# xytpai/kfunca

Measured on AMD Instinct MI355X. Metric: bf16 GEMM TFLOP/s + causal-attn fwd+bwd tokens/s, higher is better.
Workload: dtype bf16

## Files before the change

kfunca_amd/csrc/device/attention.hip:

```cpp
#include <math.h>
#include <stdlib.h>

#include <algorithm>
#include <type_traits>

#include "common.h"

namespace kf {

typedef __attribute__((ext_vector_type(8))) __bf16 bf16x8;
typedef __attribute__((ext_vector_type(8))) _Float16 f16x8;
typedef __attribute__((ext_vector_type(4))) short s16x4;
typedef __attribute__((ext_vector_type(8))) short s16x8;
typedef __attribute__((ext_vector_type(16))) float f32x16;
typedef __attribute__((ext_vector_type(4))) float f32x4;

struct AttnArgs {
    const char *q, *k, *v, *o, *d_o;
    char *out, *dq, *dk, *dv;
    float *lse;
    const float *lse_r;
    float *delta;
    float *nlse, *ndelta;
    int64_t B, H, Sq, Skv, D;
// ... 397 lines not shown
    const unsigned long long tl_loop0 = tl_t;
#endif
    for (int t = 0; t < nt; ++t) {
        const int64_t kv0 = (int64_t)t * ABK;
        TL_STAMP(6)
        asm volatile("s_waitcnt vmcnt(4)" ::: "memory");
        TL_STAMP(0)
        __builtin_amdgcn_s_barrier();
        asm volatile("" ::: "memory");
        TL_STAMP(1)
        stage(t + 2, smem + ((t + 2) % SRING) * FBUF);
        TL_STAMP(2)
        const char *cur = smem + (t % SRING) * FBUF;
        const bool skip = !active || kv0 > qw + 31 || KF_MUT(1, t == 1 && qblk == nxb - 1);
        const bool diag = kv0 + ABK - 1 > qw;
        if (late && pending) s_pv<BF, DB>(smem + ((t + SRING - 1) % SRING) * FBUF + FTILE, vo, pf, o);
        pending = false;
        TL_STAMP(5)
        if (!skip) {
            if (diag) s_qk_sm<BF, true, D>(cur, qf, ko, o, pf, m_i, l_i, c, kv0, m, hl, a.defer TL_ARGS);
            else s_qk_sm<BF, false, D>(cur, qf, ko, o, pf, m_i, l_i, c, kv0, m, hl, a.defer TL_ARGS);
            TL_STAMP(4)
            if (late) pending = true;
            else s_pv<BF, DB>(cur + FTILE, vo, pf, o);
            TL_STAMP(5)
        }
    }
#if defined(KF_ATTN_TIMELINE) && KF_ATTN_TIMELINE != 2
    if (lane == 0 && g_attn_tl) {
        unsigned long long *dst = g_attn_tl + ((size_t)blockIdx.x * 2 + (pass & 1)) * 64 + wid * 8;
        for (int i = 0; i < 7; ++i) dst[i] = tl_acc[i];
        dst[7] = (unsigned long long)nt;
    }
#endif
#ifdef KF_ATTN_TIMELINE
    const unsigned long long tl_loop1 = __builtin_amdgcn_s_memtime();
#endif
    if (late && pending) s_pv<BF, DB>(smem + ((nt + SRING - 1) % SRING) * FBUF + FTILE, vo, pf, o);
    asm volatile("s_waitcnt vmcnt(0)" ::: "memory");
    __syncthreads();
    if (active) {
        a_store_rows<BF, DB>(smem + wid * 32 * OPAD, a.out + a_head(a.lo, bh, a.H) + qw * a.lo.sr, o, 1.f / l_i, a.lo.sr);
        if (a.lse && hl == 0) a.lse[bh * a.Sq + m] = (m_i * c + __builtin_amdgcn_logf(l_i)) * kLn2;
    }
    if (a.persist) __syncthreads();
#if defined(KF_ATTN_TIMELINE) && KF_ATTN_TIMELINE == 2
    if (lane == 0 && g_attn_tl) {
        unsigned long long *dst = g_attn_tl + ((size_t)blockIdx.x * 2 + (pass & 1)) * 64 + wid * 8;
        const unsigned long long tl_end = __builtin_amdgcn_s_memtime();
        dst[0] = tl_loop0 - tl_pass0, dst[1] = tl_loop1 - tl_loop0, dst[2] = tl_end - tl_loop1;
        dst[3] = dst[4] = dst[5] = dst[6] = 0;
        dst[7] = (unsigned long long)nt;
    }
#endif
  }
}

#ifndef KF_FWD_W4_INC
#define KF_FWD_W4_INC "attn_fwd_w4.inc"
#endif
#include KF_FWD_W4_INC
template <bool BF, bool SQ, bool D64 = false>
__global__ __launch_bounds__(256) void attn_fwd_w4_kernel(const AttnArgs a) {
    static_assert(!(SQ && D64), "the scaled-query form exists for head size 128 only");
    extern __shared__ __attribute__((aligned(16))) char smem[];
    const int nxb = (int)((a.Sq + FQ - 1) / FQ);
    const int nwx = a.persist ? nxb / 2 : nxb;
    const unsigned lds = (unsigned)(uintptr_t)(const __attribute__((address_space(3))) char *)smem;
    const int wid = __builtin_amdgcn_readfirstlane(threadIdx.x >> 6);
    const int dbytes = D64 ? 128 : 256;
    const unsigned kvn = (unsigned)((a.Skv - 1) * a.lk.sr + dbytes);
    const float c = a.scale_log2e, defer = a.defer;
    const int qsr = (int)a.lq.sr, kvsr = (int)a.lk.sr, osr = (int)a.lo.sr;
#pragma nounroll
    for (unsigned vwg = blockIdx.x; vwg < a.nvwg; vwg += gridDim.x) {
    int xb0;
    int64_t bh;
    a_block_map(nwx, a.nbh, a.xcd_map, xb0, bh, vwg);
    const char *kp = a.k + a_head_kv(a.lk, bh, a.H, a.G), *vp = a.v + a_head_kv(a.lv, bh, a.H, a.G);
    const char *qh = a.q + a_head(a.lq, bh, a.H);
    char *oh = a.out + a_head(a.lo, bh, a.H);
#pragma nounroll
    for (int pass = 0; pass < (a.persist ? 2 : 1); ++pass) {
        const int xb = ((pass & 1) != (a.persist_rev != 0)) ? nxb - 1 - xb0 : xb0;
        const int qblk = nxb - 1 - xb;
        const int64_t q0 = (int64_t)qblk * FQ;
        const char *qp = qh + q0 * a.lq.sr;
        char *op = oh + q0 * a.lo.sr;
        float *lsep = a.lse ? a.lse + bh * a.Sq + q0 : nullptr;
        const int T = (int)((q0 + FQ) / ABK);
        const int64_t qrows = a.Sq - q0 < FQ ? a.Sq - q0 : FQ;
        const unsigned qn = (unsigned)((qrows - 1) * a.lq.sr + dbytes), on = (unsigned)((qrows - 1) * a.lo.sr + dbytes), lsen = (unsigned)(qrows * 4);
        int mut = -1;
#ifdef KF_MUTANT
        if (a.mutant == 1 && qblk == nxb - 1) mut = 1;
#endif
#ifdef KF_FWD_W4_STAMPS
        unsigned long long *dbg = a.dbg;
        const unsigned dbgoff = (vwg * 2 + pass) * 4 * 32;
#define KF_W4_EXTRA , [dbg] "s"(dbg), [dbgoff] "s"(dbgoff)
#else
#define KF_W4_EXTRA
#endif
#define KF_W4_OPERANDS                                                                                                              \
    [qp] "s"(qp), [kp] "s"(kp), [vp] "s"(vp), [op] "s"(op), [lsep] "s"(lsep), [qsr] "s"(qsr), [kvsr] "s"(kvsr), [osr] "s"(osr), [T] "s"(T), \
        [wid] "s"(wid), [c] "s"(c), [defer] "s"(defer), [lds] "s"(lds), [mut] "s"(mut), [kvn] "s"(kvn), [qn] "s"(qn), [on] "s"(on), [lsen] "s"(lsen) KF_W4_EXTRA
        if constexpr (D64 && BF) asm volatile(KF_FWD_W4_D64_ASM_BF16 : : KF_W4_OPERANDS : KF_FWD_W4_CLOBBERS);
        else if constexpr (D64) asm volatile(KF_FWD_W4_D64_ASM_F16 : : KF_W4_OPERANDS : KF_FWD_W4_CLOBBERS);
        else if constexpr (BF && SQ) asm volatile(KF_FWD_W4_ASM_BF16_SQ : : KF_W4_OPERANDS : KF_FWD_W4_CLOBBERS);
        else if constexpr (BF) asm volatile(KF_FWD_W4_ASM_BF16 : : KF_W4_OPERANDS : KF_FWD_W4_CLOBBERS);
        else if constexpr (SQ) asm volatile(KF_FWD_W4_ASM_F16_SQ : : KF_W4_OPERANDS : KF_FWD_W4_CLOBBERS);
        else asm volatile(KF_FWD_W4_ASM_F16 : : KF_W4_OPERANDS : KF_FWD_W4_CLOBBERS);
#undef KF_W4_OPERANDS
#undef KF_W4_EXTRA
    }
    }
}

template <bool BF, int R>
__global__ __launch_bounds__(256) void attn_delta_kernel(const char *o, const char *d_o, float *delta, int64_t nrows, const float *lse, float *nlse,
                                                         float *ndelta, float rscale, AttnArgs::Lay lo, AttnArgs::Lay ldo, int64_t S, int64_t H, int nparts, int64_t Sc) {
    const int64_t row0 = (int64_t)blockIdx.x * (16 * R) + (threadIdx.x >> 4);
    const int part = threadIdx.x & 15;
    uint4 a[R], b[R];
#pragma unroll
    for (int i = 0; i < R; ++i) {
        a[i] = b[i] = uint4{0, 0, 0, 0};
        const int64_t row = row0 + 16 * i;
        const int64_t bh = row / Sc, sq = row - bh * Sc;
        if (row < nrows && sq < S && part < nparts) {
            a[i] = *(const uint4 *)(o + a_head(lo, bh, H) + sq * lo.sr + part * 16);
            b[i] = *(const uint4 *)(d_o + a_head(ldo, bh, H) + sq * ldo.sr + part * 16);
        }
    }
#pragma unroll
    for (int i = 0; i < R; ++i) {
        const int64_t row = row0 + 16 * i;
        float acc = 0.f;
        const uint32_t aw[4] = {a[i].x, a[i].y, a[i].z, a[i].w}, bw[4] = {b[i].x, b[i].y, b[i].z, b[i].w};
#pragma unroll
        for (int j = 0; j < 4; ++j) {
            float a0, a1, b0, b1;
            if constexpr (BF) {
                a0 = __uint_as_float(aw[j] << 16); a1 = __uint_as_float(aw[j] & 0xffff0000u);
                b0 = __uint_as_float(bw[j] << 16); b1 = __uint_as_float(bw[j] & 0xffff0000u);
            } else {
                a0 = f16_to_f32(f16_t{(uint16_t)(aw[j] & 0xffff)}); a1 = f16_to_f32(f16_t{(uint16_t)(aw[j] >> 16)});
                b0 = f16_to_f32(f16_t{(uint16_t)(bw[j] & 0xffff)}); b1 = f16_to_f32(f16_t{(uint16_t)(bw[j] >> 16)});
            }
            acc += a0 * b0 + a1 * b1;
        }
        for (int msk = 8; msk > 0; msk >>= 1) acc += __shfl_xor(acc, msk, 64);
        if (row < nrows && part == 0) {
            const int64_t bh = row / Sc, sq = row - bh * Sc;
            if (sq < S) {
                delta[bh * S + sq] = acc;
                if (nlse) {
                    nlse[row] = -lse[bh * S + sq] * rscale;
                    ndelta[row] = -acc;
                }
            } else if (nlse) {
                nlse[row] = 0.f;
                ndelta[row] = 0.f;
            }
        }
    }
}

template <bool BF, bool MASK, int D>
__device__ __forceinline__ void q_tile(const char *buf, const char *doslab, const typename AFrag<BF>::type (&qf)[D / 16], const int (&ko)[D / 16],
                                       const int (&vo)[D / 32][2], f32x16 (&dq)[D / 32], float c, float lse2, float dlt, int64_t kv0, int64_t m, int hl) {
    using frag_t = typename AFrag<BF>::type;
    constexpr int DB = D / 32;
    const char *vt = buf + FTILE;
#pragma unroll
    for (int sub = 0; sub < 2; ++sub) {
        f32x16 s, dp;
#pragma unroll
        for (int e = 0; e < 16; ++e) { s[e] = 0.f; dp[e] = 0.f; }
#pragma unroll
        for (int kg = 0; kg < D / 64; ++kg) {
#pragma unroll
            for (int kk = 4 * kg; kk < 4 * kg + 4; ++kk) s = a_mfma<BF>(*(const frag_t *)(buf + sub * 32 * AROW + ko[kk]), qf[kk], s);
            __builtin_amdgcn_sched_barrier(0);
        }
#pragma unroll
        for (int kg = 0; kg < D / 64; ++kg) {
#pragma unroll
            for (int kk = 4 * kg; kk < 4 * kg + 4; ++kk)
                dp = a_mfma<BF>(*(const frag_t *)(vt + sub * 32 * AROW + ko[kk]), *(const frag_t *)(doslab + ko[kk]), dp);
            __builtin_amdgcn_sched_barrier(0);
        }
#pragma unroll
        for (int e = 0; e < 16; ++e) {
            float p = __builtin_amdgcn_exp2f(__builtin_fmaf(s[e], c, -lse2));
            if (MASK && kv0 + sub * 32 + a_row(e, hl) > m) p = 0.f;
            s[e] = p * (dp[e] - dlt);
        }
        TrN<DB> ta;
        if (sub == 0) tr4_issue<0>(buf, vo, ta); else tr4_issue<32 * AROW>(buf, vo, ta);
        tr4_wait1(ta);
        { const frag_t df = a_pack<BF>(s, 0);
#pragma unroll
          for (int d = 0; d < DB; ++d) dq[d] = a_mfma<BF>(tr4_frag<BF, DB>(ta, d), df, dq[d]); }
        __builtin_amdgcn_sched_barrier(0);
        if (sub == 0) tr4_issue<16 * AROW>(buf, vo, ta); else tr4_issue<48 * AROW>(buf, vo, ta);
        tr4_wait1(ta);
        { const frag_t df = a_pack<BF>(s, 1);
#pragma unroll
          for (int d = 0; d < DB; ++d) dq[d] = a_mfma<BF>(tr4_frag<BF, DB>(ta, d), df, dq[d]); }
        __builtin_amdgcn_sched_barrier(0);
    }
}

constexpr int QSLAB = 32 * AROW;
constexpr int QLDS = FRING * FBUF + 8 * QSLAB;

template <bool BF, int D>
__global__ __launch_bounds__(FNT, 2) void attn_bwd_dq_v2_kernel(const AttnArgs a) {
    using frag_t = typename AFrag<BF>::type;
    constexpr int KS = D / 16, DB = D / 32;
    extern __shared__ __attribute__((aligned(16))) char smem[];
    const int lane = threadIdx.x & 63, wid = threadIdx.x >> 6, xl = lane & 31, hl = lane >> 5;
    int xb0;
    int64_t bh;
    const int nxb = (int)((a.Sq + FQ - 1) / FQ);
    const int nwx = a.persist ? nxb / (2 * a.persist) : nxb;
    a_block_map(nwx, a.nbh, a.xcd_map, xb0, bh);
    const char *Kg = a.k + a_head_kv(a.lk, bh, a.H, a.G);
    const char *Vg = a.v + a_head_kv(a.lv, bh, a.H, a.G);
    char *doslab = smem + FRING * FBUF + wid * QSLAB;
    int ko[KS], vo[DB][2];
#pragma unroll
    for (int kk = 0; kk < KS; ++kk) ko[kk] = a_off(xl, kk * 2 + hl);
#pragma unroll
    for (int d = 0; d < DB; ++d) {
        vo[d][0] = a_tr_lane_off(d * 32, 0);
        vo[d][1] = a_tr_lane_off(d * 32, 1);
    }
    const float c = a.scale * kLog2e;
#pragma nounroll
  for (int pass = 0; pass < (a.persist ? 2 * a.persist : 1); ++pass) {
    const int xp = xb0 + (pass >> 1) * nwx;
    const int xb = ((pass & 1) != (a.persist_rev != 0)) ? nxb - 1 - xp : xp;
    const int qblk = nxb - 1 - xb;
    const int64_t q0 = (int64_t)qblk * FQ, qw = q0 + wid * 32, m = qw + xl;
    const bool active = qw < a.Sq;

    frag_t qf[KS];
    float lse2 = 0.f, dlt = 0.f;
    if (active) {
        const char *Qg = a.q + a_head(a.lq, bh, a.H) + m * a.lq.sr;
#pragma unroll
        for (int kk = 0; kk < KS; ++kk) qf[kk] = *(const frag_t *)(Qg + (kk * 16 + 8 * hl) * 2);
        const char *dOw = a.d_o + a_head(a.ldo, bh, a.H) + qw * a.ldo.sr;
#pragma unroll
        for (int i = 0; i < 8; ++i)
            if (D == AD || ((lane + 64 * i) & 15) < D / 8) a_lst(doslab, lane + 64 * i, a_gld(dOw, lane + 64 * i, a.ldo.sr));
        lse2 = a.lse_r[bh * a.Sq + m] * kLog2e;
        dlt = a.delta[bh * a.Sq + m];
    } else {
#pragma unroll
        for (int kk = 0; kk < KS; ++kk)
#pragma unroll
            for (int j = 0; j < 8; ++j) qf[kk][j] = 0;
    }
    f32x16 dq[DB];
#pragma unroll
    for (int d = 0; d < DB; ++d)
#pragma unroll
        for (int e = 0; e < 16; ++e) dq[d][e] = 0.f;

    const int64_t q_end = q0 + FQ < a.Sq ? q0 + FQ : a.Sq;
    const int64_t kv_end = a.Skv < q_end ? a.Skv : q_end;
    const int nt = (int)((kv_end + ABK - 1) / ABK);
    auto stage = [&](int tile, char *buf) {
        const int64_t kv = (int64_t)(tile < nt ? tile : nt - 1) * ABK;
        f_stage<D>(Kg + kv * a.lk.sr, Vg + kv * a.lv.sr, buf, a.lk.sr, a.lv.sr);
    };
    asm volatile("s_waitcnt vmcnt(0) lgkmcnt(0)" ::: "memory");
    stage(0, smem);
    stage(1, smem + FBUF);
    for (int t = 0; t < nt; ++t) {
        const int64_t kv0 = (int64_t)t * ABK;
        asm volatile("s_waitcnt vmcnt(4)" ::: "memory");
        __builtin_amdgcn_s_barrier();
        asm volatile("" ::: "memory");
        stage(t + 2, smem + ((t + 2) % FRING) * FBUF);
        const char *cur = smem + (t % FRING) * FBUF;
        const bool skip = !active || kv0 > qw + 31 || KF_MUT(4, t == 0 && qblk == nxb - 1);
        const bool diag = kv0 + ABK - 1 > qw;
        if (!skip) {
            if (diag) q_tile<BF, true, D>(cur, doslab, qf, ko, vo, dq, c, lse2, dlt, kv0, m, hl);
            else q_tile<BF, false, D>(cur, doslab, qf, ko, vo, dq, c, lse2, dlt, kv0, m, hl);
        }
    }
    asm volatile("s_waitcnt vmcnt(0)" ::: "memory");
    __syncthreads();
    if (active) a_store_rows<BF, DB>(smem + wid * 32 * OPAD, a.dq + a_head(a.ldq, bh, a.H) + qw * a.ldq.sr, dq, a.scale, a.ldq.sr);
    if (a.persist) __syncthreads();
  }
}

constexpr int DQ_RING = 3;
constexpr int DQ_SLAB = 2 * DS_TILE;
constexpr int DQ_LDS = DQ_RING * FTILE + 8 * DQ_RING * DQ_SLAB;

template <bool BF, int HF, int KS, int DB>
__device__ __forceinline__ void dq_step(const char *kt, const int (&vo)[DB][2], unsigned dsb, f32x16 (&dq)[DB]) {
    s16x4 blo, bhi;
    TrN<DB> ta;
    asm volatile("ds_read_b64_tr_b16 %0, %2 offset:%c3\n\tds_read_b64_tr_b16 %1, %2 offset:%c4"
                 : "=&v"(blo), "=&v"(bhi)
                 : "v"(dsb), "n"(HF * DS_TILE + KS * 512), "n"(HF * DS_TILE + KS * 512 + 256)
                 : "memory");
    tr4_issue<(32 * HF + 16 * KS) * AROW>(kt, vo, ta);
    asm volatile("s_waitcnt lgkmcnt(0)" : "+v"(blo), "+v"(bhi) : : "memory");
    tr4_wait1(ta);
    s16x8 r;
    r[0] = blo[0]; r[1] = blo[1]; r[2] = blo[2]; r[3] = blo[3];
    r[4] = bhi[0]; r[5] = bhi[1]; r[6] = bhi[2]; r[7] = bhi[3];
    const auto b = __builtin_bit_cast(typename AFrag<BF>::type, r);
#pragma unroll
    for (int d = 0; d < DB; ++d) dq[d] = a_mfma<BF>(tr4_frag<BF, DB>(ta, d), b, dq[d]);
}

template <bool BF, int D>
__global__ __launch_bounds__(FNT, 2) void attn_bwd_dq_ds_kernel(const AttnArgs a) {
    constexpr int DB = D / 32;
    extern __shared__ __attribute__((aligned(16))) char smem[];
    const int lane = threadIdx.x & 63, wid = __builtin_amdgcn_readfirstlane(threadIdx.x >> 6);
    int xb0;
    int64_t bh;
    const int nxb = (int)((a.Sq + FQ - 1) / FQ);
    const int nwx = a.persist ? nxb / (2 * a.persist) : nxb;
    a_block_map(nwx, a.nbh, a.xcd_map, xb0, bh);
    bh += a.bh0;
    const char *Kg = a.k + a_head_kv(a.lk, bh, a.H, a.G);
    char *slab = smem + DQ_RING * FTILE + wid * DQ_RING * DQ_SLAB;
    int vo[DB][2];
#pragma unroll
    for (int d = 0; d < DB; ++d) {
        vo[d][0] = a_tr_lane_off(d * 32, 0);
        vo[d][1] = a_tr_lane_off(d * 32, 1);
    }
    const int grp = lane >> 4, qq = (lane >> 2) & 3, pp = lane & 3, h = grp >> 1;
    const unsigned smem_u = (unsigned)(uintptr_t)(const __attribute__((address_space(3))) char *)smem;
    const int sp = grp & 1;
    const unsigned ds_rd = smem_u + (unsigned)(slab - smem) + sp * 1024 + 64 * ((2 * h + (qq >> 1)) ^ (2 * sp)) + 32 * (qq & 1) + 16 * (pp & 1) + 8 * (pp >> 1);
    int ds_src[2];
#pragma unroll
    for (int pc = 0; pc < 2; ++pc) ds_src[pc] = pc * 1024 + (((lane >> 2) ^ (2 * pc)) * 4 + (lane & 3)) * 16;
    const int krow = lane >> 4, kpos = lane & 15;
#pragma nounroll
  for (int pass = 0; pass < (a.persist ? 2 * a.persist : 1); ++pass) {
    const int xp = xb0 + (pass >> 1) * nwx;
    const int xb = ((pass & 1) != (a.persist_rev != 0)) ? nxb - 1 - xp : xp;
    const int qblk = nxb - 1 - xb;
    const int64_t q0 = (int64_t)qblk * FQ, qw = q0 + wid * 32;
    const bool active = qw < a.Sq;
    const int sl = (int)(qw >> 5);
    f32x16 dq[DB];
#pragma unroll
    for (int d = 0; d < DB; ++d)
#pragma unroll
        for (int e = 0; e < 16; ++e) dq[d][e] = 0.f;
    const int64_t q_end = q0 + FQ < a.Sq ? q0 + FQ : a.Sq;
    const int64_t kv_end = a.Skv < q_end ? a.Skv : q_end;
    const int nt = (int)((kv_end + ABK - 1) / ABK);
    const char *dsg = a.ds + ((bh - a.bh0) * a.ds_pair + ds_row_base(qblk, a.ds_nkb, a.ds_tri) + wid) * DS_TILE;
    const int kwb_last = (int)(a.ds_nkb * 8 - 1);
    const int slw = qblk * 8 + wid;
    auto stage = [&](int tile, int slot) {
        const int tl = tile < nt ? tile : nt - 1;
        const int kfirst = tl * ABK, klast = (int)a.Skv - 1 - kfirst;
        const char *kg = Kg + (int64_t)kfirst * a.lk.sr;
#pragma unroll
        for (int i = 0; i < 2; ++i) {
            const int row0 = (wid * 2 + i) * 4, row = row0 + krow;
            const int chunk = kpos ^ (((row & 3) << 2) | ((row >> 2) & 3));
            const int srow = row < klast ? row : klast;
            if (D == AD || chunk < D / 8)
                __builtin_amdgcn_global_load_lds((const __attribute__((address_space(1))) void *)(kg + (int64_t)srow * a.lk.sr + chunk * 16),
                                                 (__attribute__((address_space(3))) void *)(smem + slot * FTILE + row0 * AROW), 16, 0, 0);
        }
#pragma unroll
        for (int hf = 0; hf < 2; ++hf) {
            int kwb = 2 * tl + hf;
            kwb = kwb < kwb_last ? kwb : kwb_last;
            kwb = kwb <= slw ? kwb : (slw < kwb_last ? slw : kwb_last);
            const char *tg = dsg + (int64_t)kwb * 8 * DS_TILE;
#pragma unroll
            for (int pc = 0; pc < 2; ++pc)
                __builtin_amdgcn_global_load_lds((const __attribute__((address_space(1))) void *)(tg + ds_src[pc]),
                                                 (__attribute__((address_space(3))) void *)(slab + slot * DQ_SLAB + hf * DS_TILE + pc * 1024), 16, 0, 0);
        }
    };
    stage(0, 0);
    stage(1, 1);
    for (int t = 0; t < nt; ++t) {
        asm volatile("s_waitcnt vmcnt(6)" ::: "memory");
        __builtin_amdgcn_s_barrier();
        asm volatile("" ::: "memory");
        stage(t + 2, (t + 2) % DQ_RING);
        const char *kt = smem + (t % DQ_RING) * FTILE;
        const unsigned dsb = ds_rd + (unsigned)((t % DQ_RING) * DQ_SLAB);
        if (active && 2 * t <= sl && !KF_MUT(3, t == 0 && qblk == nxb - 1)) {
            dq_step<BF, 0, 0, DB>(kt, vo, dsb, dq);
            dq_step<BF, 0, 1, DB>(kt, vo, dsb, dq);
            if (2 * t + 1 <= sl) {
                dq_step<BF, 1, 0, DB>(kt, vo, dsb, dq);
                dq_step<BF, 1, 1, DB>(kt, vo, dsb, dq);
            }
        }
    }
    asm volatile("s_waitcnt vmcnt(0)" ::: "memory");
    __syncthreads();
    if (active) a_store_rows<BF, DB>(smem + wid * 32 * OPAD, a.dq + a_head(a.ldq, bh, a.H) + qw * a.ldq.sr, dq, a.scale, a.ldq.sr,
                                     (int)(a.Sq - qw < 32 ? a.Sq - qw : 32));
    if (a.persist) __syncthreads();
  }
}

constexpr int BQS = 32;

constexpr int K4B = 128;
constexpr int K4SL = 2 * BQS * AROW + 256;
constexpr int K4PAIR = 2 * K4SL;
constexpr int K4LDS = 4 * K4PAIR;
constexpr bool K4_SPREAD = true;
static_assert(K4LDS >= 4 * 32 * OPAD, "epilogue slabs must fit");

template <int OFF>
__device__ __forceinline__ void k4_rows4(unsigned e, unsigned o, s16x8 (&f)[4]) {
    asm volatile("ds_read_b128 %0, %4 offset:%c6\n\tds_read_b128 %1, %5 offset:%c6\n\t"
                 "ds_read_b128 %2, %4 offset:%c7\n\tds_read_b128 %3, %5 offset:%c7"
                 : "=&v"(f[0]), "=&v"(f[1]), "=&v"(f[2]), "=&v"(f[3])
                 : "v"(e), "v"(o), "n"(OFF), "n"(OFF + 512)
                 : "memory");
}
template <int OFF>
__device__ __forceinline__ void k4_rowc(unsigned lr, f32x4 (&c)[4]) {
    asm volatile("ds_read_b128 %0, %4 offset:%c5\n\tds_read_b128 %1, %4 offset:%c6\n\t"
                 "ds_read_b128 %2, %4 offset:%c7\n\tds_read_b128 %3, %4 offset:%c8"
                 : "=&a"(c[0]), "=&a"(c[1]), "=&a"(c[2]), "=&a"(c[3])
                 : "v"(lr), "n"(OFF), "n"(OFF + 32), "n"(OFF + 64), "n"(OFF + 96)
                 : "memory");
}
struct K4Tr { s16x4 lo[4], hi[4]; };
template <int OFF>
__device__ __forceinline__ void k4_tr4(unsigned t0, unsigned t1, K4Tr &t) {
    asm volatile("ds_read_b64_tr_b16 %0, %8 offset:%c10\n\tds_read_b64_tr_b16 %1, %9 offset:%c10\n\t"
                 "ds_read_b64_tr_b16 %2, %8 offset:%c11\n\tds_read_b64_tr_b16 %3, %9 offset:%c11\n\t"
                 "ds_read_b64_tr_b16 %4, %8 offset:%c12\n\tds_read_b64_tr_b16 %5, %9 offset:%c12\n\t"
                 "ds_read_b64_tr_b16 %6, %8 offset:%c13\n\tds_read_b64_tr_b16 %7, %9 offset:%c13"
                 : "=&v"(t.lo[0]), "=&v"(t.hi[0]), "=&v"(t.lo[1]), "=&v"(t.hi[1]), "=&v"(t.lo[2]), "=&v"(t.hi[2]), "=&v"(t.lo[3]), "=&v"(t.hi[3])
                 : "v"(t0), "v"(t1), "n"(OFF), "n"(OFF + 512), "n"(OFF + 1024), "n"(OFF + 1536)
                 : "memory");
}
template <int N>
__device__ __forceinline__ void k4_wait4(s16x8 (&f)[4]) {
    asm volatile("s_waitcnt lgkmcnt(%c4)" : "+v"(f[0]), "+v"(f[1]), "+v"(f[2]), "+v"(f[3]) : "n"(N) : "memory");
}
template <int N>
__device__ __forceinline__ void k4_wait4c(s16x8 (&f)[4], f32x4 (&c)[4]) {
    asm volatile("s_waitcnt lgkmcnt(%c8)"
                 : "+v"(f[0]), "+v"(f[1]), "+v"(f[2]), "+v"(f[3]), "+a"(c[0]), "+a"(c[1]), "+a"(c[2]), "+a"(c[3])
                 : "n"(N)
                 : "memory");
}
template <int N>
__device__ __forceinline__ void k4_wait_tr(K4Tr &a) {
    asm volatile("s_waitcnt lgkmcnt(%c8)"
                 : "+v"(a.lo[0]), "+v"(a.hi[0]), "+v"(a.lo[1]), "+v"(a.hi[1]), "+v"(a.lo[2]), "+v"(a.hi[2]), "+v"(a.lo[3]), "+v"(a.hi[3])
                 : "n"(N)
                 : "memory");
}
template <bool BF>
__device__ __forceinline__ typename AFrag<BF>::type k4_frag(const K4Tr &t, int d) {
    s16x8 r;
    r[0] = t.lo[d][0]; r[1] = t.lo[d][1]; r[2] = t.lo[d][2]; r[3] = t.lo[d][3];
    r[4] = t.hi[d][0]; r[5] = t.hi[d][1]; r[6] = t.hi[d][2]; r[7] = t.hi[d][3];
    return __builtin_bit_cast(typename AFrag<BF>::type, r);
}
__device__ __forceinline__ f32x16 k4_acc(const f32x4 (&c)[4]) {
    f32x16 r;
#pragma unroll
    for (int g = 0; g < 4; ++g)
#pragma unroll
        for (int j = 0; j < 4; ++j) r[4 * g + j] = c[g][j];
    return r;
}

template <int OFF>
__device__ __forceinline__ void k4_rows4a(unsigned e, unsigned o, s16x8 (&f)[4]) {
    asm volatile("ds_read_b128 %0, %4 offset:%c6\n\tds_read_b128 %1, %5 offset:%c6\n\t"
                 "ds_read_b128 %2, %4 offset:%c7\n\tds_read_b128 %3, %5 offset:%c7"
                 : "=&a"(f[0]), "=&a"(f[1]), "=&a"(f[2]), "=&a"(f[3])
                 : "v"(e), "v"(o), "n"(OFF), "n"(OFF + 512)
                 : "memory");
}
template <int OFF>
__device__ __forceinline__ void k4_rowcv(unsigned lr, f32x4 (&c)[4]) {
    asm volatile("ds_read_b128 %0, %4 offset:%c5\n\tds_read_b128 %1, %4 offset:%c6\n\t"
                 "ds_read_b128 %2, %4 offset:%c7\n\tds_read_b128 %3, %4 offset:%c8"
                 : "=&v"(c[0]), "=&v"(c[1]), "=&v"(c[2]), "=&v"(c[3])
                 : "v"(lr), "n"(OFF), "n"(OFF + 32), "n"(OFF + 64), "n"(OFF + 96)
                 : "memory");
}
template <int N>
__device__ __forceinline__ void k4_wait4a_cv(s16x8 (&f)[4], f32x4 (&c)[4]) {
    asm volatile("s_waitcnt lgkmcnt(%c8)"
                 : "+a"(f[0]), "+a"(f[1]), "+a"(f[2]), "+a"(f[3]), "+v"(c[0]), "+v"(c[1]), "+v"(c[2]), "+v"(c[3])
                 : "n"(N)
                 : "memory");
}
template <int N>
__device__ __forceinline__ void k4_wait4a(s16x8 (&f)[4]) {
    asm volatile("s_waitcnt lgkmcnt(%c4)" : "+a"(f[0]), "+a"(f[1]), "+a"(f[2]), "+a"(f[3]) : "n"(N) : "memory");
}
template <int N>
__device__ __forceinline__ void k4_wait4_cv(s16x8 (&f)[4], f32x4 (&c)[4]) {
    asm volatile("s_waitcnt lgkmcnt(%c8)"
                 : "+v"(f[0]), "+v"(f[1]), "+v"(f[2]), "+v"(f[3]), "+v"(c[0]), "+v"(c[1]), "+v"(c[2]), "+v"(c[3])
                 : "n"(N)
                 : "memory");
}
template <int OFF>
__device__ __forceinline__ void k4_row1(unsigned a, s16x8 &f) { asm volatile("ds_read_b128 %0, %1 offset:%c2" : "=&v"(f) : "v"(a), "n"(OFF) : "memory"); }
template <int OFF>
__device__ __forceinline__ void k4_row1a(unsigned a, s16x8 &f) { asm volatile("ds_read_b128 %0, %1 offset:%c2" : "=&a"(f) : "v"(a), "n"(OFF) : "memory"); }
template <int OFF>
__device__ __forceinline__ void k4_rowc1(unsigned lr, f32x4 &c) { asm volatile("ds_read_b128 %0, %1 offset:%c2" : "=&v"(c) : "v"(lr), "n"(OFF) : "memory"); }
template <int OFF>
__device__ __forceinline__ void k4_trp(unsigned t0, unsigned t1, s16x4 &lo, s16x4 &hi) {
    asm volatile("ds_read_b64_tr_b16 %0, %2 offset:%c4\n\tds_read_b64_tr_b16 %1, %3 offset:%c4" : "=&v"(lo), "=&v"(hi) : "v"(t0), "v"(t1), "n"(OFF) : "memory");
}
template <bool BF, bool AA>
__device__ __forceinline__ void k4_mfma_first(f32x16 &acc, s16x8 &a, const typename AFrag<BF>::type &b, f32x16 &c) {
    if constexpr (BF) {
        if constexpr (AA) asm volatile("s_nop 1\n\tv_mfma_f32_32x32x16_bf16 %0, %1, %3, %2" : "=&v"(acc), "+a"(a), "+v"(c) : "a"(b));
        else asm volatile("s_nop 1\n\tv_mfma_f32_32x32x16_bf16 %0, %1, %3, %2" : "=&v"(acc), "+v"(a), "+v"(c) : "a"(b));
    } else {
        if constexpr (AA) asm volatile("s_nop 1\n\tv_mfma_f32_32x32x16_f16 %0, %1, %3, %2" : "=&v"(acc), "+a"(a), "+v"(c) : "a"(b));
        else asm volatile("s_nop 1\n\tv_mfma_f32_32x32x16_f16 %0, %1, %3, %2" : "=&v"(acc), "+v"(a), "+v"(c) : "a"(b));
    }
}
template <bool BF, bool AA>
__device__ __forceinline__ void k4_mfma_acc(f32x16 &acc, s16x8 &a, const typename AFrag<BF>::type &b) {
    if constexpr (BF) {
        if constexpr (AA) asm volatile("v_mfma_f32_32x32x16_bf16 %0, %1, %2, %0" : "+v"(acc), "+a"(a) : "a"(b));
        else asm volatile("v_mfma_f32_32x32x16_bf16 %0, %1, %2, %0" : "+v"(acc), "+v"(a) : "a"(b));
    } else {
        if constexpr (AA) asm volatile("v_mfma_f32_32x32x16_f16 %0, %1, %2, %0" : "+v"(acc), "+a"(a) : "a"(b));
        else asm volatile("v_mfma_f32_32x32x16_f16 %0, %1, %2, %0" : "+v"(acc), "+v"(a) : "a"(b));
    }
}
template <bool BF>
__device__ __forceinline__ void k4_mfma_first_t(f32x16 &acc, s16x8 &a, const typename AFrag<BF>::type &b, f32x16 &c, f32x16 &tag) {
    if constexpr (BF) asm volatile("s_nop 1\n\tv_mfma_f32_32x32x16_bf16 %0, %1, %4, %2\n\ts_nop 3" : "=&v"(acc), "+v"(a), "+v"(c), "+v"(tag) : "a"(b));
    else asm volatile("s_nop 1\n\tv_mfma_f32_32x32x16_f16 %0, %1, %4, %2\n\ts_nop 3" : "=&v"(acc), "+v"(a), "+v"(c), "+v"(tag) : "a"(b));
}
template <bool BF>
__device__ __forceinline__ void k4_mfma_acc_t(f32x16 &acc, s16x8 &a, const typename AFrag<BF>::type &b, f32x16 &tag) {
    if constexpr (BF) asm volatile("v_mfma_f32_32x32x16_bf16 %0, %1, %3, %0" : "+v"(acc), "+v"(a), "+v"(tag) : "a"(b));
    else asm volatile("v_mfma_f32_32x32x16_f16 %0, %1, %3, %0" : "+v"(acc), "+v"(a), "+v"(tag) : "a"(b));
}
__device__ __forceinline__ void k4_keep(s16x8 (&f)[4]) { asm volatile("" : "+v"(f[0]), "+v"(f[1]), "+v"(f[2]), "+v"(f[3])); }
__device__ __forceinline__ void k4_keep(f32x16 &c) { asm volatile("" : "+v"(c)); }

template <int OFF>
__device__ __forceinline__ void k4_tr2(unsigned t0, unsigned t1, K4Tr &t) {
    asm volatile("ds_read_b64_tr_b16 %0, %4 offset:%c6\n\tds_read_b64_tr_b16 %1, %5 offset:%c6\n\t"
                 "ds_read_b64_tr_b16 %2, %4 offset:%c7\n\tds_read_b64_tr_b16 %3, %5 offset:%c7"
                 : "=&v"(t.lo[0]), "=&v"(t.hi[0]), "=&v"(t.lo[1]), "=&v"(t.hi[1])
                 : "v"(t0), "v"(t1), "n"(OFF), "n"(OFF + 512)
                 : "memory");
}
template <int N>
__device__ __forceinline__ void k4_wait_tr2(K4Tr &a) {
    asm volatile("s_waitcnt lgkmcnt(%c4)" : "+v"(a.lo[0]), "+v"(a.hi[0]), "+v"(a.lo[1]), "+v"(a.hi[1]) : "n"(N) : "memory");
}

__device__ __forceinline__ float k4_mul(float a, float b) { return a * b; }
__device__ __forceinline__ float k4_mul_odd(float a, float b) { return __builtin_fmaf(a, b, 0.f); }
#ifdef KF_ABL_DKV_NOVALU
#define KF_ABL_EXP(x) (x)
#define KF_ABL_MUL(a, b) (b)
#define KF_ABL_MUL_ODD(a, b) (b)
#else
#define KF_ABL_EXP(x) __builtin_amdgcn_exp2f(x)
#define KF_ABL_MUL(a, b) k4_mul(a, b)
#define KF_ABL_MUL_ODD(a, b) k4_mul_odd(a, b)
#endif
template <bool BF, bool DS, int D>
__global__ __launch_bounds__(256) void attn_bwd_dkv_v4_kernel(const AttnArgs a) {
    using frag_t = typename AFrag<BF>::type;
    constexpr int KS = D / 16, DB = D / 32;
    extern __shared__ __attribute__((aligned(16))) char smem[];
    const int lane = threadIdx.x & 63, wid = __builtin_amdgcn_readfirstlane(threadIdx.x >> 6), xl = lane & 31, hl = lane >> 5;
    int xb0;
    int64_t bh;
    const int nkb = (int)(a.Skv / K4B), nwx = a.persist ? nkb / (2 * a.persist) : nkb;
    a_block_map(nwx, a.nbh, a.xcd_map, xb0, bh);
    bh += a.bh0;
    const char *Qg = a.q + a_head(a.lq, bh, a.H);
    const char *dOg = a.d_o + a_head(a.ldo, bh, a.H);
    const char *Kh = a.k + a_head_kv(a.lk, bh, a.H, a.G), *Vh = a.v + a_head_kv(a.lv, bh, a.H, a.G);
#pragma nounroll
  for (int pass = 0; pass < (a.persist ? 2 * a.persist : 1); ++pass) {
    const int xp = xb0 + (pass >> 1) * nwx;
    const int xb = ((pass & 1) != (a.persist_rev != 0)) ? nkb - 1 - xp : xp;
    const int64_t k0 = (int64_t)xb * K4B, kw = k0 + wid * 32, n = kw + xl;
#ifdef KF_ATTN_TIMELINE
    const unsigned long long tl_pass0 = __builtin_amdgcn_s_memtime();
#endif

    frag_t kf[8], vf[8];
    const float c = a.scale * kLog2e;
    {
        const char *Kg = Kh + n * a.lk.sr;
        const char *Vg = Vh + n * a.lv.sr;
#pragma unroll
        for (int kk = 0; kk < KS; ++kk) {
            kf[kk] = *(const frag_t *)(Kg + (kk * 16 + 8 * hl) * 2);
            vf[kk] = *(const frag_t *)(Vg + (kk * 16 + 8 * hl) * 2);
        }
    }
    f32x16 dk[4], dv[4];
#pragma unroll
    for (int d = 0; d < DB; ++d)
#pragma unroll
        for (int e = 0; e < 16; ++e) { dk[d][e] = 0.f; dv[d][e] = 0.f; }

    const unsigned smem_u = (unsigned)(uintptr_t)(const __attribute__((address_space(3))) char *)smem;
    const int rsw = (xl >> 2) & 3;
    const unsigned rb_e = smem_u + 2048 * (xl >> 3) + 64 * (xl & 7) + 16 * ((0 + hl) ^ rsw);
    const unsigned rb_o = smem_u + 2048 * (xl >> 3) + 64 * (xl & 7) + 16 * ((2 + hl) ^ rsw);
    const int g = lane >> 4, qq = (lane & 15) >> 2, pp = lane & 3, h = g >> 1;
    const int tslot = 2 * (g & 1) + (pp >> 1);
    const unsigned tb_0 = smem_u + 64 * (4 * h + qq) + 16 * (tslot ^ h) + 8 * (pp & 1);
    const unsigned tb_1 = smem_u + 2048 + 64 * (4 * h + qq) + 16 * (tslot ^ (h + 2)) + 8 * (pp & 1);
    const unsigned lr = smem_u + 2 * BQS * AROW + 16 * hl;

    int64_t soffq[2], soffd[2];
#pragma unroll
    for (int i = 0; i < 2; ++i) {
        const int sub = 2 * i + (lane >> 5), r = (lane >> 2) & 7, slot = lane & 3, row = 8 * wid + r;
        const int ch = (4 * sub + (slot ^ ((row >> 2) & 3))) * 16;
        soffq[i] = row * a.lq.sr + ch;
        soffd[i] = row * a.ldo.sr + ch;
    }
    const float *rcg = lane < BQS ? a.nlse + bh * a.Sqc + lane : a.ndelta + bh * a.Sqc + lane - BQS;
    const int ns = (int)(a.Sq / BQS), np = ns / 2;
    unsigned ds_lane = (unsigned)(xl * 32 + hl * 16);
    const char *ds_base = DS ? a.ds + ((bh - a.bh0) * a.ds_pair + (kw >> 5) * 8) * DS_TILE : nullptr;
    const int ds_nkb = (int)a.ds_nkb, ds_tri = a.ds_tri;
    auto stage_piece = [&](auto id_c, int pr_, int slot4) __attribute__((always_inline)) {
        constexpr int ID = decltype(id_c)::value, SL = ID / 5, K = ID % 5;
        if constexpr (D == 64 && (K == 2 || K == 3)) return;
        const int prc = pr_ < np ? pr_ : np - 1;
        const int64_t qs_ = ((int64_t)prc * 2 + SL) * BQS;
        char *buf = smem + slot4 * K4PAIR + SL * K4SL;
        if constexpr (K == 4) {
            __builtin_amdgcn_global_load_lds((const __attribute__((address_space(1))) void *)(rcg + qs_),
                                             (__attribute__((address_space(3))) void *)(buf + 2 * BQS * AROW), 4, 0, 0);
        } else {
            constexpr int i = K >> 1;
            const char *src = (K & 1) ? dOg + qs_ * a.ldo.sr + soffd[i] : Qg + qs_ * a.lq.sr + soffq[i];
            __builtin_amdgcn_global_load_lds((const __attribute__((address_space(1))) void *)src,
                                             (__attribute__((address_space(3))) void *)(buf + (K & 1) * BQS * AROW + 1024 * (2 * wid + i)), 16, 0, 0);
        }
    };
    auto stage_pair = [&](int pr_, int slot4) __attribute__((always_inline)) {
        stage_piece(std::integral_constant<int, 0>{}, pr_, slot4); stage_piece(std::integral_constant<int, 1>{}, pr_, slot4);
        stage_piece(std::integral_constant<int, 2>{}, pr_, slot4); stage_piece(std::integral_constant<int, 3>{}, pr_, slot4);
        stage_piece(std::integral_constant<int, 4>{}, pr_, slot4); stage_piece(std::integral_constant<int, 5>{}, pr_, slot4);
        stage_piece(std::integral_constant<int, 6>{}, pr_, slot4); stage_piece(std::integral_constant<int, 7>{}, pr_, slot4);
        stage_piece(std::integral_constant<int, 8>{}, pr_, slot4); stage_piece(std::integral_constant<int, 9>{}, pr_, slot4);
    };

    const int p0 = (int)(k0 / (2 * BQS));
    stage_pair(p0, 0);
    stage_pair(p0 + 1, 1);
    stage_pair(p0 + 2, 2);
    {
#pragma unroll
        for (int kk = 0; kk < KS; ++kk) asm volatile("" : "+a"(kf[kk]), "+a"(vf[kk]));
    }
    if constexpr (D == 128) asm volatile("s_waitcnt vmcnt(10)" ::: "memory");
    else asm volatile("s_waitcnt vmcnt(6)" ::: "memory");
    __builtin_amdgcn_s_barrier();
    asm volatile("" ::: "memory");

#ifdef KF_ATTN_TIMELINE
    unsigned long long tlk[10], tlk_acc[11] = {0, 0, 0, 0, 0, 0, 0, 0, 0, 0, 0}, tlk_prev = __builtin_amdgcn_s_memtime();
#endif
    s16x8 g0[4], g1[4];
    f32x4 cs[4], cp[4];
    if constexpr (D == 128) {
        k4_rowcv<0>(lr, cs);
        k4_rows4a<0>(rb_e, rb_o, g0);
        k4_rows4a<1024>(rb_e, rb_o, g1);
        k4_rowcv<128>(lr, cp);
    } else {
        k4_rowcv<0>(lr, cs);
        k4_rows4a<0>(rb_e, rb_o, g0);
        k4_rowcv<128>(lr, cp);
        k4_rows4<BQS * AROW>(rb_e, rb_o, g1);
    }

#define K4_MFMA4(ACC, FR, BOP, K0)                                                                                   \
    _Pragma("unroll") for (int kk = 0; kk < 4; ++kk) ACC = a_mfma<BF>(__builtin_bit_cast(frag_t, FR[kk]), BOP[K0 + kk], ACC);
#define K4_CVT2(DST, J, A, B)                                              \
    if constexpr (BF) { DST[J] = (__bf16)(A); DST[(J) + 1] = (__bf16)(B); } \
    else { DST[J] = (_Float16)(A); DST[(J) + 1] = (_Float16)(B); }
// ... 1521 lines not shown
```

Measured before the change: 7.654 million.

## Decouple K and dS prefetch rings in dQ kernel with deeper dS lead

Splits the combined K/dS staging in the dQ backward kernel into separate rings: K uses a 2-slot ring with lead 1, while dS half-tiles use an 8-slot ring prefetched 3 tiles ahead, with the second half's load issued between the two MFMA halves. The vmcnt wait is derived from the new lead depths. The aim is to hide dS global-load latency better, which dominates this memory-bound kernel, while shrinking K LDS usage. The risk is a shallower K prefetch exposing K latency, and changed LDS footprint affecting occupancy.

Measured after the change: 7.678 million, median of 3. About the same (+0.3%).

```diff
diff --git a/kfunca_amd/csrc/device/attention.hip b/kfunca_amd/csrc/device/attention.hip
--- a/kfunca_amd/csrc/device/attention.hip
+++ b/kfunca_amd/csrc/device/attention.hip
@@ -723,9 +723,17 @@
   }
 }
 
-constexpr int DQ_RING = 3;
-constexpr int DQ_SLAB = 2 * DS_TILE;
-constexpr int DQ_LDS = DQ_RING * FTILE + 8 * DQ_RING * DQ_SLAB;
+constexpr int DQ_KRING = 2;
+constexpr int DQ_KLEAD = DQ_KRING - 1;
+constexpr int DQ_DSLEAD = 3;
+constexpr int DQ_DSRING = 2 * DQ_DSLEAD + 2;
+constexpr int DQ_DS_CPOL = 0;
+constexpr int DQ_LDS = DQ_KRING * FTILE + 8 * DQ_DSRING * DS_TILE;
+constexpr int DQ_VMCNT = 4 + 6 * (DQ_KLEAD - 1) < 6 * (DQ_DSLEAD - 1) ? 4 + 6 * (DQ_KLEAD - 1) : 6 * (DQ_DSLEAD - 1);
+static_assert(DQ_KRING >= 2 && DQ_DSRING >= 2 * DQ_DSLEAD + 1, "a slot is refilled only after its tile was consumed");
+static_assert(DQ_LDS <= 160 * 1024, "the dQ kernel's rings must fit the CU's LDS");
+static_assert(DQ_LDS >= 8 * 32 * OPAD, "epilogue slabs must fit");
+static_assert(DQ_VMCNT >= 0 && DQ_VMCNT < 64, "s_waitcnt vmcnt is a 6-bit count");
 
 template <bool BF, int HF, int KS, int DB>
 __device__ __forceinline__ void dq_step(const char *kt, const int (&vo)[DB][2], unsigned dsb, f32x16 (&dq)[DB]) {
@@ -733,7 +741,7 @@
     TrN<DB> ta;
     asm volatile("ds_read_b64_tr_b16 %0, %2 offset:%c3\n\tds_read_b64_tr_b16 %1, %2 offset:%c4"
                  : "=&v"(blo), "=&v"(bhi)
-                 : "v"(dsb), "n"(HF * DS_TILE + KS * 512), "n"(HF * DS_TILE + KS * 512 + 256)
+                 : "v"(dsb), "n"(KS * 512), "n"(KS * 512 + 256)
                  : "memory");
     tr4_issue<(32 * HF + 16 * KS) * AROW>(kt, vo, ta);
     asm volatile("s_waitcnt lgkmcnt(0)" : "+v"(blo), "+v"(bhi) : : "memory");
@@ -758,7 +766,7 @@
     a_block_map(nwx, a.nbh, a.xcd_map, xb0, bh);
     bh += a.bh0;
     const char *Kg = a.k + a_head_kv(a.lk, bh, a.H, a.G);
-    char *slab = smem + DQ_RING * FTILE + wid * DQ_RING * DQ_SLAB;
+    char *slab = smem + DQ_KRING * FTILE + wid * DQ_DSRING * DS_TILE;
     int vo[DB][2];
 #pragma unroll
     for (int d = 0; d < DB; ++d) {
@@ -792,10 +800,11 @@
     const char *dsg = a.ds + ((bh - a.bh0) * a.ds_pair + ds_row_base(qblk, a.ds_nkb, a.ds_tri) + wid) * DS_TILE;
     const int kwb_last = (int)(a.ds_nkb * 8 - 1);
     const int slw = qblk * 8 + wid;
-    auto stage = [&](int tile, int slot) {
+    auto stage_k = [&](int tile) {
         const int tl = tile < nt ? tile : nt - 1;
         const int kfirst = tl * ABK, klast = (int)a.Skv - 1 - kfirst;
         const char *kg = Kg + (int64_t)kfirst * a.lk.sr;
+        char *kslot = smem + (tile % DQ_KRING) * FTILE;
 #pragma unroll
         for (int i = 0; i < 2; ++i) {
             const int row0 = (wid * 2 + i) * 4, row = row0 + krow;
@@ -803,36 +812,44 @@
             const int srow = row < klast ? row : klast;
             if (D == AD || chunk < D / 8)
                 __builtin_amdgcn_global_load_lds((const __attribute__((address_space(1))) void *)(kg + (int64_t)srow * a.lk.sr + chunk * 16),
-                                                 (__attribute__((address_space(3))) void *)(smem + slot * FTILE + row0 * AROW), 16, 0, 0);
-        }
-#pragma unroll
-        for (int hf = 0; hf < 2; ++hf) {
-            int kwb = 2 * tl + hf;
-            kwb = kwb < kwb_last ? kwb : kwb_last;
-            kwb = kwb <= slw ? kwb : (slw < kwb_last ? slw : kwb_last);
-            const char *tg = dsg + (int64_t)kwb * 8 * DS_TILE;
-#pragma unroll
-            for (int pc = 0; pc < 2; ++pc)
-                __builtin_amdgcn_global_load_lds((const __attribute__((address_space(1))) void *)(tg + ds_src[pc]),
-                                                 (__attribute__((address_space(3))) void *)(slab + slot * DQ_SLAB + hf * DS_TILE + pc * 1024), 16, 0, 0);
+                                                 (__attribute__((address_space(3))) void *)(kslot + row0 * AROW), 16, 0, 0);
         }
     };
-    stage(0, 0);
-    stage(1, 1);
+    auto stage_ds = [&](int tile, int hf) {
+        const int tl = tile < nt ? tile : nt - 1;
+        int kwb = 2 * tl + hf;
+        kwb = kwb < kwb_last ? kwb : kwb_last;
+        kwb = kwb <= slw ? kwb : (slw < kwb_last ? slw : kwb_last);
+        const char *tg = dsg + (int64_t)kwb * 8 * DS_TILE;
+        char *dslot = slab + ((2 * tile + hf) % DQ_DSRING) * DS_TILE;
+#pragma unroll
+        for (int pc = 0; pc < 2; ++pc)
+            __builtin_amdgcn_global_load_lds((const __attribute__((address_space(1))) void *)(tg + ds_src[pc]),
+                                             (__attribute__((address_space(3))) void *)(dslot + pc * 1024), 16, 0, DQ_DS_CPOL);
+    };
+#pragma unroll
+    for (int s = -DQ_DSLEAD; s < 0; ++s) {
+        if (s + DQ_KLEAD >= 0) stage_k(s + DQ_KLEAD);
+        stage_ds(s + DQ_DSLEAD, 0);
+        stage_ds(s + DQ_DSLEAD, 1);
+    }
     for (int t = 0; t < nt; ++t) {
-        asm volatile("s_waitcnt vmcnt(6)" ::: "memory");
+        asm volatile("s_waitcnt vmcnt(%c0)" ::"n"(DQ_VMCNT) : "memory");
         __builtin_amdgcn_s_barrier();
         asm volatile("" ::: "memory");
-        stage(t + 2, (t + 2) % DQ_RING);
-        const char *kt = smem + (t % DQ_RING) * FTILE;
-        const unsigned dsb = ds_rd + (unsigned)((t % DQ_RING) * DQ_SLAB);
-        if (active && 2 * t <= sl && !KF_MUT(3, t == 0 && qblk == nxb - 1)) {
-            dq_step<BF, 0, 0, DB>(kt, vo, dsb, dq);
-            dq_step<BF, 0, 1, DB>(kt, vo, dsb, dq);
-            if (2 * t + 1 <= sl) {
-                dq_step<BF, 1, 0, DB>(kt, vo, dsb, dq);
-                dq_step<BF, 1, 1, DB>(kt, vo, dsb, dq);
-            }
+        stage_k(t + DQ_KLEAD);
+        stage_ds(t + DQ_DSLEAD, 0);
+        const char *kt = smem + (t % DQ_KRING) * FTILE;
+        const unsigned ds0 = ds_rd + (unsigned)(((2 * t) % DQ_DSRING) * DS_TILE), ds1 = ds_rd + (unsigned)(((2 * t + 1) % DQ_DSRING) * DS_TILE);
+        const bool on = active && 2 * t <= sl && !KF_MUT(3, t == 0 && qblk == nxb - 1);
+        if (on) {
+            dq_step<BF, 0, 0, DB>(kt, vo, ds0, dq);
+            dq_step<BF, 0, 1, DB>(kt, vo, ds0, dq);
+        }
+        stage_ds(t + DQ_DSLEAD, 1);
+        if (on && 2 * t + 1 <= sl) {
+            dq_step<BF, 1, 0, DB>(kt, vo, ds1, dq);
+            dq_step<BF, 1, 1, DB>(kt, vo, ds1, dq);
         }
     }
     asm volatile("s_waitcnt vmcnt(0)" ::: "memory");
```
